# ubc-vision/DiffuseSG

Hardware: NVIDIA B200
Metric: sampled scene graphs/sec (higher is better)
Workload: dtype bf16

## Files before the change

### diffusesg_b200/csrc/gemm.cu

```cuda
#include "common.cuh"
#include "kernels.h"

namespace dsg {
namespace {

constexpr int BM = 128;
constexpr int BK = 64;
__host__ __device__ constexpr int epi_groups(int epi) { return (epi == EPI_RES_F32 || epi == EPI_F32) ? 2 : 4; }
__host__ __device__ constexpr int gemm_threads(int epi) { return 64 + 128 * epi_groups(epi); }
constexpr int A_STAGE_BYTES = BM * BK * 2;

template <int BN, bool PAIR = false>
struct Cfg {
  static constexpr int kStages = PAIR ? ((BN == 256) ? 4 : (BN == 192) ? 5 : 7) : ((BN == 256) ? 3 : (BN == 192) ? 4 : 5);
  static constexpr int B_STAGE_BYTES = (PAIR ? BN / 2 : BN) * BK * 2;
  static constexpr int STAGE_BYTES = A_STAGE_BYTES + B_STAGE_BYTES;
  static constexpr int ACC_STRIDE = (BN >= 192) ? 256 : 128;
  static constexpr uint32_t TMEM_COLS = 2 * ACC_STRIDE;
  static constexpr int STAGING_BYTES = 64 * 1024;
  static constexpr int BIAS_BYTES = 2 * BN * 4;
  static constexpr int SMEM_BYTES = 1024  + kStages * STAGE_BYTES + STAGING_BYTES + BIAS_BYTES + 256 ;
};

static_assert(Cfg<96>::SMEM_BYTES <= 227 * 1024 && Cfg<192>::SMEM_BYTES <= 227 * 1024, "shared memory budget");
// ... 159 lines not shown
      else mbar_arrive(&tempty_bar[acc]);
    };
    for (int tile = cta + acc * ncta; tile < num_tiles; tile += 2 * ncta) {
      const int mn = tile / ksplit;
      const int m_blk = PAIR ? (mn / num_n) * 2 + static_cast<int>(rank) : mn / num_n;
      const int n_blk = mn % num_n;
      const uint32_t t_row = tmem_base + (static_cast<uint32_t>(q * 32) << 16) + acc * C::ACC_STRIDE;
      if (EPI == EPI_ADJ_HEAD) {
        float* sPart = reinterpret_cast<float*>(sOut) + acc * 128 * 8;
        if (tile == cta + acc * ncta) {
          if (tig < 48) sBiasA[half * 48 + tig] = p.bias[half * 48 + tig];
          asm volatile("bar.sync %0, 128;" ::"r"(bar_id) : "memory");
        }
        const int row = m_blk * BM + r_in_tile;
        const int n_ = p.n_img, nn_ = n_ * n_;
        const int rowc = row < p.M ? row : p.M - 1;
        int b_ = rowc / nn_, ij_ = rowc - b_ * nn_;
        if (p.perm != nullptr) {
          const int ss = p.side * p.side;
          const int img = rowc / ss, rem = rowc - img * ss;
          const int ii = rem / p.side;
          b_ = p.perm[img];
          ij_ = ii * n_ + (rem - ii * p.side);
        }
        const bool real_ = b_ >= 0;
        if (!real_) b_ = 0;
        bool ok_ = false;
        float cs_ = 0.f, co_ = 1.f, xa_[8];
        if (half == 0) {
          const int i_ = ij_ / n_, j_ = ij_ - i_ * n_;
          ok_ = p.flags[b_ * n_ + i_] != 0 && p.flags[b_ * n_ + j_] != 0;
          if (p.x_adj != nullptr) {
            cs_ = p.c_skip[b_];
            co_ = p.c_out[b_];
#pragma unroll
            for (int c = 0; c < 8; ++c) xa_[c] = c < p.c_e ? p.x_adj[(static_cast<size_t>(b_) * p.c_e + c) * nn_ + ij_] : 0.f;
          }
        }
        mbar_wait(&tfull_bar[acc], acc_ph);
        tcgen05_fence_after();
        f32x2 y2[4] = {f2_splat(0.f), f2_splat(0.f), f2_splat(0.f), f2_splat(0.f)};
#pragma unroll
        for (int c0 = 0; c0 < 48; c0 += 16) {
          uint32_t r[16];
          tmem_ld_32x16(t_row + half * 48 + c0, r);
// ... 328 lines not shown
bool gemm_use_pair(long long rows, int K, int epi) {
  return epi != EPI_ADJ_HEAD && rows >= 256 && (K >= 768 || (K >= 384 && epi == EPI_BF16));
}

int launch_gemm(const CUtensorMap* tmA, const CUtensorMap* tmW, const CUtensorMap* tmO, int epi, const GemmParams& p,
                cudaStream_t st, bool pair) {
  DSG_REQUIRE(p.M > 0 && p.N > 0 && p.K > 0 && p.N % 96 == 0 && p.K % 16 == 0,
              "gemm: unsupported shape M=%d N=%d K=%d (N %% 96 == 0 and K %% 16 == 0 required)", p.M, p.N, p.K);
  DSG_REQUIRE(p.out != nullptr, "gemm: null output");
  DSG_REQUIRE(p.ksplit <= 1, "gemm: split-K (ksplit %d) is only for the MN-major weight-gradient GEMM", p.ksplit);
  const int bn = p.bn ? p.bn : gemm_block_n(p.N);
  DSG_REQUIRE(p.N % bn == 0 && (bn == 96 || bn == 192 || bn == 256), "gemm: tile width %d for N = %d", bn, p.N);
  if (epi == EPI_ADJ_HEAD) {
    DSG_REQUIRE(p.N == 96 && p.c_e >= 1 && p.c_e <= 8 && p.w2t && p.b2 && p.flags && p.n_img > 0,
                "gemm: adj-head epilogue needs N == 96, c_e <= 8 and the head tensors");
    return launch_t<96, EPI_ADJ_HEAD>(tmA, tmW, tmO, p, st);
  }
  DSG_REQUIRE(p.ldo % 8 == 0, "gemm: ldo must be a multiple of 8");
  DSG_REQUIRE(tmO != nullptr && p.ldo == p.N, "gemm: output tensor map missing or ldo != N");
  if (epi == EPI_RES_F32)
    DSG_REQUIRE(p.res == p.out, "gemm: the residual epilogue accumulates in place (res must alias out)");
  if (pair) {
    if (bn == 256) {
      switch (epi) {
        case EPI_BF16: return launch_pair<256, EPI_BF16>(tmA, tmW, tmO, p, st);
        case EPI_GELU_BF16: return launch_pair<256, EPI_GELU_BF16>(tmA, tmW, tmO, p, st);
        case EPI_RES_F32: return launch_pair<256, EPI_RES_F32>(tmA, tmW, tmO, p, st);
        case EPI_F32: return launch_pair<256, EPI_F32>(tmA, tmW, tmO, p, st);
      }
    } else if (bn == 192) {
// ... 43 lines not shown
```

### diffusesg_b200/csrc/kernels.h

```cpp
#pragma once

#include <cuda.h>
#include <cuda_bf16.h>
#include <cuda_runtime.h>
#include <stdint.h>

namespace dsg {

typedef __nv_bfloat16 bf16;

enum GemmEpi : int {
  EPI_BF16 = 0,
  EPI_GELU_BF16 = 1,
  EPI_RES_F32 = 2,
  EPI_F32 = 3,
  EPI_ADJ_HEAD = 4,
};

struct GemmParams {
  int M, N, K;
  const float* bias;
  const float* res;
  void* out;
  int ldo;
  int bn;
  int ksplit;
  int scale_rows;
  float row_scale;
  const float* w2t;
  const float* b2;
  int c_e;
  int n_img;
  const uint8_t* flags;
  const float* x_adj;
  const float* c_skip;
  const float* c_out;
  const int* perm;
  int side;
};

int make_tmap_bf16(CUtensorMap* map, const void* base, int64_t rows, int64_t cols, int box_rows);
int make_tmap_out(CUtensorMap* map, const void* base, int64_t rows, int64_t cols, int epi);

int launch_wgrad(const void* dy, const void* x, float* dw, long long tokens, int n_out, int x_cols, int out_cols, int ksplit,
                 int scale_rows, float row_scale, cudaStream_t st);

int gemm_block_n(int N);
int gemm_choose_bn(long long rows, int N, int K, int epi, bool pair);
bool gemm_use_pair(long long rows, int K, int epi);
int launch_gemm(const CUtensorMap* tmA, const CUtensorMap* tmW, const CUtensorMap* tmO, int epi, const GemmParams& p,
                cudaStream_t st, bool pair = false);

bool fused_mlp_supported(int C);
// ... 49 lines not shown
int launch_breakup_ln(const float* t, bf16* y, const float* g1, const float* b1, const float* g2, const float* b2,
                      int batch, int res, int D, cudaStream_t st, const int* tok0 = nullptr, const int* width = nullptr,
                      int sh = 0, const int* src_perm = nullptr);

int launch_cond(const float* noise_labels, long long label_stride, int n_cond, const float* w0, const float* b0, const float* w1,
                const float* b1, const float* w_film, const float* b_film, int film_total, float* emb0, float* emb1,
                float* emb, float* film, int embed, cudaStream_t st);

int launch_precond_coef(const float* sigmas, int sigma_stride, float* coef, int batch, cudaStream_t st);

int launch_node_proj(const float* node, const float* sc_node, const float* in_scale, const float* w_rc,
                     float* rc, int batch, int n, int c_n, int self_cond, int embed, cudaStream_t st);
int launch_patch_embed(const float* adj, const float* sc_adj, const float* in_scale, const uint8_t* flags,
                       const float* rc, const float* w_adj, const float* bias, const float* gamma,
                       const float* beta, const float* film, int film_ld, int film_off, int cond_uniform,
                       float* x0, int batch, int n, int c_e, int self_cond, int embed, cudaStream_t st,
                       const int* perm = nullptr, int side = 0);
int launch_node_head(const bf16* rep, const uint8_t* flags, const float* fold_t, const float* fold_b, const float* w1t,
                     const float* b1, const float* w2t, const float* b2, const float* x_node, const float* c_skip, const float* c_out,
                     float* out_node, int batch, int n, int c_n, int embed, cudaStream_t st, const int* tok0 = nullptr,
                     const int* width = nullptr, float* scratch = nullptr);


int launch_edm_pre_step(const float* adj, const float* node, const float* eps_adj, const float* eps_node,
                        const uint8_t* flags, float noise_coef, float* adj_hat, float* node_hat, int batch,
                        int c_e, int n, int c_n, cudaStream_t st);
int launch_edm_pre_step_philox(const float* adj, const float* node, const uint8_t* flags, float noise_coef,
                               unsigned long long seed, unsigned long long offset_adj, int grid_adj,
                               unsigned long long offset_node, int grid_node, const void* dev_params, float* adj_hat,
                               float* node_hat, int batch, int c_e, int n, int c_n, cudaStream_t st);
int launch_edm_post_step(const float* adj_hat, const float* node_hat, const float* d1_adj, const float* d1_node,
                         const float* d2_adj, const float* d2_node, const uint8_t* flags, float inv_t_hat,
// ... 35 lines not shown
```

### diffusesg_b200/csrc/model.cu

```cuda
#include <cstdarg>
#include <cstdio>
#include <cstdlib>
#include <cstring>
#include <map>
#include <string>
#include <tuple>
#include <vector>

#include "../../include/dsg_b200.h"
#include "common.cuh"
#include "kernels.h"

namespace dsg {

static thread_local char g_err[1024] = "";
static unsigned long long g_launches = 0;
static int g_stop_after = -1;

void set_last_error(const char* fmt, ...) {
  va_list ap;
  va_start(ap, fmt);
  vsnprintf(g_err, sizeof(g_err), fmt, ap);
  va_end(ap);
}
// ... 370 lines not shown
  std::vector<float*> skip;
  bf16 *Y, *QKV, *ATT, *H;
  size_t bytes;
};

struct Layout {
  int level = 0;
  int K = 0;
  int count[8], side[8], img0[8];
  long long tok[9];
  const int *perm = nullptr, *tok0 = nullptr, *width = nullptr;
  bool dense() const { return perm == nullptr; }
  const int* bucket_perm(int k) const { return perm != nullptr ? perm + img0[k] : nullptr; }
  long long tokens(int s) const { return tok[K] >> (2 * s); }
  long long at(int k, int s) const { return tok[k] >> (2 * s); }
};

Layout dense_layout(int B, int N) {
  Layout l;
  l.K = 1;
  l.count[0] = B; l.side[0] = N; l.img0[0] = 0;
  l.tok[0] = 0; l.tok[1] = static_cast<long long>(B) * N * N;
  return l;
}

int parse_plan(Layout& c, int level, const int32_t* tables, int table_images, int buckets, const int32_t* counts,
               const int32_t* sides, long long phantom_tok0, int G, int B, int N) {
  DSG_REQUIRE(buckets > 0 && buckets <= 8 && table_images > 0, "forward: %d buckets", buckets);
  c.level = level;
  c.K = buckets;
// ... 433 lines not shown
  bool final_ln_done = false;
  auto block = [&](const Block& b, const float* x_in, const Layout& from, const Layout& lay, bool last) -> int {
    const int* rows_map = row_map(a, from, lay);
    if (rows_map != nullptr && x_in == w.X) std::swap(w.X, w.T);
    return run_block(m, b, w, x_in, lay, rows_map, uniform, st, last, &final_ln_done);
  };
  g_prof_pass = g_prof_on && !stream_capturing(st) && (g_prof_counter++ % g_prof_stride == 0);
  struct ProfPassGuard { ~ProfPassGuard() { g_prof_pass = false; } } prof_pass_guard;
  DSG_TRY_P(PC_EMBED_HEAD, 0, 0, launch_cond(labels, label_stride, a->n_cond, m->f32("map_layer0.weight"),
                      m->f32("map_layer0.bias"), m->f32("map_layer1.weight"), m->f32("map_layer1.bias"),
                      m->at<float>(m->film_w_off), m->at<float>(m->film_b_off), m->film_total, w.emb0, w.emb1, w.emb,
                      w.film, E, st));
  DSG_TRY_P(PC_EMBED_HEAD, 0, 0, launch_node_proj(a->node, a->sc_node, c_in, m->at<float>(m->w_rc_off), w.rc, B, N, m->cfg.c_n,
                           m->cfg.self_condition, E, st));
  const Layout& l0 = stage_layout(0);
  for (int k = 0; k < l0.K; ++k) {
    const double pxk = static_cast<double>(l0.count[k]) * l0.side[k] * l0.side[k];
    DSG_TRY_P(PC_EMBED_HEAD, 0, pxk * (m->planes_adj * 4 + E * 4),
              launch_patch_embed(a->adj, a->sc_adj, c_in, a->flags, w.rc, m->at<float>(m->w_adj_off),
                                 m->f32("patch_embed.proj.bias"), m->f32("patch_embed.norm.weight"),
                                 m->f32("patch_embed.norm.bias"), w.film, m->film_total, 0, uniform, w.X + l0.tok[k] * E,
                                 l0.count[k], N, m->cfg.c_e, m->cfg.self_condition, E, st, l0.bucket_perm(k), l0.side[k]));
  }
  const Layout* xl = &l0;
  int stage_no = 0;
#define DSG_STAGE_DONE() do { if (g_stop_after >= 0 && stage_no++ == g_stop_after) return DSG_OK; } while (0)
  DSG_STAGE_DONE();
  for (int s = 0; s < m->nl; ++s) {
    const float* x_in = s == 0 ? w.X : w.skip[s - 1];
    const Layout* in = s == 0 ? xl : &stage_layout(s - 1);
    for (int j = 0; j < m->cfg.depths[s]; ++j) {
      const Layout& lay = block_layout(s, j, 0);
      DSG_TRY(block(m->blocks[m->down_first[s] + j], x_in, *in, lay, false));
      x_in = w.X;
      in = xl = &lay;
      DSG_STAGE_DONE();
    }
    if (s < m->nl - 1) {
// ... 43 lines not shown
  const long long pixels = l0.tokens(0);
  if (!l0.dense())
    DSG_CUDA_CHECK(cudaMemsetAsync(a->out_adj, 0, static_cast<size_t>(B) * m->cfg.c_e * N * N * 4, st));
  if (!final_ln_done)
    DSG_TRY_P(PC_ROW, 0, static_cast<double>(pixels) * E * 6, launch_ln(w.X, w.Y, m->f32("norm.weight"), m->f32("norm.bias"), pixels, E, st));
  GemmParams hp;
  memset(&hp, 0, sizeof(hp));
  hp.w2t = m->at<float>(m->adj_w2t_off);
  hp.b2 = m->at<float>(m->adj_b2_off);
  hp.c_e = m->cfg.c_e;
  hp.n_img = N;
  hp.flags = a->flags;
  hp.x_adj = a->mode == 1 ? a->adj : nullptr;
  hp.c_skip = c_skip;
  hp.c_out = c_out;
  for (int k = 0; k < l0.K; ++k) {
    hp.perm = l0.bucket_perm(k);
    hp.side = l0.side[k];
    DSG_TRY(gemm(m, w.Y + l0.tok[k] * E, l0.tok[k + 1] - l0.tok[k], m->adj_fc1, EPI_ADJ_HEAD, m->at<float>(m->adj_b1_off),
                 nullptr, a->out_adj, st, &hp));
  }
  DSG_TRY_P(PC_EMBED_HEAD, 0, static_cast<double>(pixels) * E * 2, launch_node_head(w.Y, a->flags, m->at<float>(m->fold_ft_off), m->at<float>(m->fold_b_off),
                           m->at<float>(m->node_w1t_off), m->f32("readout_node_mlp.fc1.bias"),
                           m->at<float>(m->node_w2t_off), m->f32("readout_node_mlp.fc2.bias"),
                           a->mode == 1 ? a->node : nullptr, c_skip, c_out, a->out_node, B, N, m->cfg.c_n, E, st,
                           l0.tok0, l0.width, 2 * E >= 128 ? w.rc : nullptr));
  return DSG_OK;
}

void dsg_launch_count_add(uint64_t n) { __atomic_fetch_add(&g_launches, static_cast<unsigned long long>(n), __ATOMIC_RELAXED); }
void dsg_debug_set_stop_after(int n_stages) { g_stop_after = n_stages; }

int dsg_profile_begin(int pass_stride) {
  DSG_REQUIRE(pass_stride >= 1, "profile_begin: stride %d", pass_stride);
  for (int c = 0; c < PC_COUNT; ++c) {
    memset(&g_prof_tot[c], 0, sizeof(g_prof_tot[c]));
// ... 245 lines not shown
```

### diffusesg_b200/csrc/rowops.cu

```cuda
#include "common.cuh"
#include "kernels.h"

namespace dsg {
namespace {

constexpr int kRowThreads = 256;
constexpr float kLnEps = 1e-5f;

DSG_DEVICE uint2 pack4_bf16(float a, float b, float c, float d) { return make_uint2(pack_bf16x2(a, b), pack_bf16x2(c, d)); }

template <int LPR>
DSG_DEVICE float group_sum(float v) {
#pragma unroll
  for (int o = LPR / 2; o > 0; o >>= 1) v += __shfl_xor_sync(0xffffffffu, v, o);
  return v;
}

template <int NV, int LPR = 32>
struct Row {
  float4 v[NV];
  DSG_DEVICE void load(const float* p, int C, int lane) {
#pragma unroll
    for (int i = 0; i < NV; ++i) {
      const int e = (lane + LPR * i) * 4;
// ... 284 lines not shown
  if (e2 >= 2 * embed) return;
  const int which = e2 / embed, e = e2 - which * embed;
  const float* w = w_rc + static_cast<size_t>(which) * cin * embed + e;
  float wr[32];
#pragma unroll
  for (int ch = 0; ch < 32; ++ch) wr[ch] = ch < cin ? w[ch * embed] : 0.f;
  for (int r = 0; r < kNodeRows && row0 + r < rows; ++r) {
    float acc = 0.f;
#pragma unroll
    for (int ch = 0; ch < 32; ++ch) acc = fmaf(wr[ch], sv[r][ch], acc);
    rc[(row0 + r) * 2 * embed + e2] = acc;
  }
}

constexpr int kPE = 96;
__global__ void __launch_bounds__(kRowThreads, 3)
patch_embed_kernel(const float* __restrict__ adj, const float* __restrict__ sc_adj, const float* __restrict__ in_scale,
                   const uint8_t* __restrict__ flags, const float* __restrict__ rc, const float* __restrict__ w_adj,
                   const float* __restrict__ bias, const float* __restrict__ gamma, const float* __restrict__ beta,
                   const float* __restrict__ film, int film_ld, int cond_uniform, float* __restrict__ x0,
                   long long pixels, int n, int c_e, int self_cond, const int* __restrict__ perm, int side) {
  constexpr int E = kPE, NT = E / 8;
  __shared__ uint4 sBf[NT][32];
  __shared__ __align__(16) float sBias[E], sGam[E], sBet[E];
  const int planes = self_cond ? 2 * c_e : c_e;
  const int lane = threadIdx.x & 31, g = lane >> 2, t = lane & 3;
  auto split2 = [](float a, float b, uint32_t& hi, uint32_t& lo) {
    const __nv_bfloat16 ah = __float2bfloat16_rn(a), bh = __float2bfloat16_rn(b);
    hi = pack_bf16x2(__bfloat162float(ah), __bfloat162float(bh));
    lo = pack_bf16x2(a - __bfloat162float(ah), b - __bfloat162float(bh));
  };
  for (int idx = threadIdx.x; idx < NT * 32; idx += kRowThreads) {
    const int nt = idx >> 5, l = idx & 31, ch = nt * 8 + (l >> 2), k0 = 2 * (l & 3);
    auto w = [&](int k) { return k < planes ? w_adj[k * E + ch] : 0.f; };
    uint4 f;
    split2(w(k0), w(k0 + 1), f.x, f.z);
    split2(w(k0 + 8), w(k0 + 9), f.y, f.w);
    sBf[nt][l] = f;
  }
  for (int i = threadIdx.x; i < E; i += kRowThreads) { sBias[i] = bias[i]; sGam[i] = gamma[i]; sBet[i] = beta[i]; }
  __syncthreads();
  const int nn = n * n;
  const long long groups = (pixels + 15) / 16;
  const long long warps_total = static_cast<long long>(gridDim.x) * (kRowThreads / 32);
  auto load_planes = [&](long long grp, float (&pv)[8], float (&scl)[2]) {
#pragma unroll
    for (int r = 0; r < 2; ++r) {
      const long long px = grp * 16 + g + 8 * r;
      const long long pc = px < pixels ? px : pixels - 1;
      int b_ = static_cast<int>(pc / nn);
      int ij_ = static_cast<int>(pc - static_cast<long long>(b_) * nn);
      if (perm != nullptr) {
        const int img = static_cast<int>(pc / (side * side));
        const int rem = static_cast<int>(pc - static_cast<long long>(img) * side * side);
        const int i_ = rem / side;
        b_ = perm[img];
        ij_ = i_ * n + (rem - i_ * side);
      }
      scl[r] = (in_scale && b_ >= 0) ? in_scale[b_] : 1.f;
      if (b_ < 0) {
#pragma unroll
        for (int h = 0; h < 4; ++h) pv[r * 4 + h] = 0.f;
        continue;
      }
#pragma unroll
      for (int h = 0; h < 4; ++h) {
        const int k = 2 * t + (h & 1) + 8 * (h >> 1);
        float a = 0.f;
        if (k < planes) {
          if (self_cond && k < c_e) {
            if (sc_adj) a = sc_adj[(static_cast<size_t>(b_) * c_e + k) * nn + ij_];
          } else {
            a = adj[(static_cast<size_t>(b_) * c_e + (self_cond ? k - c_e : k)) * nn + ij_];
          }
        }
        pv[r * 4 + h] = a;
      }
    }
  };
  const long long grp0 = static_cast<long long>(blockIdx.x) * (kRowThreads / 32) + (threadIdx.x >> 5);
  float pv_next[8], sc_next[2];
  if (grp0 < groups) load_planes(grp0, pv_next, sc_next);
  for (long long grp = grp0; grp < groups; grp += warps_total) {
    float pv[8];
#pragma unroll
    for (int k = 0; k < 8; ++k) {
      const int kk = 2 * t + (k & 1) + 8 * ((k >> 1) & 1);
      pv[k] = (self_cond && kk < c_e) ? pv_next[k] : __fmul_rn(sc_next[k >> 2], pv_next[k]);
    }
    if (grp + warps_total < groups) load_planes(grp + warps_total, pv_next, sc_next);
    long long pix[2];
    int bb[2], ij[2];
    bool valid[2], pair_ok[2];
    const float *rrow[2], *rcol[2], *fs[2];
#pragma unroll
    for (int r = 0; r < 2; ++r) {
      pix[r] = grp * 16 + g + 8 * r;
      valid[r] = pix[r] < pixels;
      const long long pc = valid[r] ? pix[r] : pixels - 1;
      bb[r] = static_cast<int>(pc / nn);
      ij[r] = static_cast<int>(pc - static_cast<long long>(bb[r]) * nn);
      if (perm != nullptr) {
        const int img = static_cast<int>(pc / (side * side));
        const int rem = static_cast<int>(pc - static_cast<long long>(img) * side * side);
        const int ii = rem / side;
        bb[r] = perm[img];
        ij[r] = ii * n + (rem - ii * side);
      }
      const int i_ = ij[r] / n, j_ = ij[r] - i_ * n;
      const int bs = bb[r] < 0 ? 0 : bb[r];
      pair_ok[r] = bb[r] >= 0 && flags[bs * n + i_] != 0 && flags[bs * n + j_] != 0;
      rrow[r] = rc + (static_cast<size_t>(bs) * n + i_) * 2 * E;
      rcol[r] = rc + (static_cast<size_t>(bs) * n + j_) * 2 * E + E;
      fs[r] = film + static_cast<size_t>(cond_uniform ? 0 : bs) * film_ld;
    }
    uint32_t a_hi[4], a_lo[4];
    split2(pv[0], pv[1], a_hi[0], a_lo[0]);
    split2(pv[4], pv[5], a_hi[1], a_lo[1]);
    split2(pv[2], pv[3], a_hi[2], a_lo[2]);
    split2(pv[6], pv[7], a_hi[3], a_lo[3]);
    float acc[NT][4];
#pragma unroll
    for (int nt = 0; nt < NT; ++nt) {
      const float2 bv = *reinterpret_cast<const float2*>(&sBias[nt * 8 + 2 * t]);
      acc[nt][0] = bv.x; acc[nt][1] = bv.y; acc[nt][2] = bv.x; acc[nt][3] = bv.y;
      const uint4 f = sBf[nt][lane];
      const uint32_t b_hi[2] = {f.x, f.y}, b_lo[2] = {f.z, f.w};
      mma_m16n8k16_bf16(acc[nt], a_lo, b_hi);
      mma_m16n8k16_bf16(acc[nt], a_hi, b_lo);
      mma_m16n8k16_bf16(acc[nt], a_hi, b_hi);
    }
    f32x2 pr[NT][2];
#pragma unroll
    for (int nt = 0; nt < NT; ++nt) {
      pr[nt][0] = f2_pack(acc[nt][0], acc[nt][1]);
      pr[nt][1] = f2_pack(acc[nt][2], acc[nt][3]);
    }
    float mean[2], rstd[2];
#pragma unroll
    for (int r = 0; r < 2; ++r) {
      if (pair_ok[r]) {
        const float2* p1 = reinterpret_cast<const float2*>(rrow[r] + 2 * t);
        const float2* p2 = reinterpret_cast<const float2*>(rcol[r] + 2 * t);
#pragma unroll
        for (int nt = 0; nt < NT; ++nt) {
          const float2 r1 = __ldg(p1 + 4 * nt), r2 = __ldg(p2 + 4 * nt);
          pr[nt][r] = f2_add(pr[nt][r], f2_add(f2_pack(r1.x, r1.y), f2_pack(r2.x, r2.y)));
        }
      }
      f32x2 s2 = pr[0][r];
#pragma unroll
      for (int nt = 1; nt < NT; ++nt) s2 = f2_add(s2, pr[nt][r]);
      float sa, sb;
      f2_unpack(s2, sa, sb);
      float sm = sa + sb;
      sm += __shfl_xor_sync(0xffffffffu, sm, 1);
      sm += __shfl_xor_sync(0xffffffffu, sm, 2);
      mean[r] = sm * (1.0f / E);
      const f32x2 nm = f2_splat(-mean[r]);
      f32x2 q2 = f2_splat(0.f);
#pragma unroll
      for (int nt = 0; nt < NT; ++nt) {
        pr[nt][r] = f2_add(pr[nt][r], nm);
        q2 = f2_fma(pr[nt][r], pr[nt][r], q2);
      }
      f2_unpack(q2, sa, sb);
      float qq = sa + sb;
      qq += __shfl_xor_sync(0xffffffffu, qq, 1);
      qq += __shfl_xor_sync(0xffffffffu, qq, 2);
      rstd[r] = rsqrtf(qq * (1.0f / E) + kLnEps);
    }
#pragma unroll
    for (int r = 0; r < 2; ++r) {
      const f32x2 rs = f2_splat(rstd[r]);
      const float2* psc = reinterpret_cast<const float2*>(fs[r] + 2 * t);
      const float2* psh = reinterpret_cast<const float2*>(fs[r] + E + 2 * t);
      float2* orow = reinterpret_cast<float2*>(x0 + pix[r] * E + 2 * t);
      if (valid[r]) {
#pragma unroll
        for (int nt = 0; nt < NT; ++nt) {
          const float2 gg = *reinterpret_cast<const float2*>(&sGam[nt * 8 + 2 * t]);
          const float2 be = *reinterpret_cast<const float2*>(&sBet[nt * 8 + 2 * t]);
          const float2 fsc = __ldg(psc + 4 * nt), fsh = __ldg(psh + 4 * nt);
          const f32x2 y = f2_fma(f2_mul(pr[nt][r], rs), f2_pack(gg.x, gg.y), f2_pack(be.x, be.y));
          const f32x2 z = f2_fma(y, f2_add(f2_pack(fsc.x, fsc.y), f2_splat(1.f)), f2_pack(fsh.x, fsh.y));
          float z0, z1, u0, u1;
          f2_unpack(z, z0, z1);
          f2_unpack(f2_mul(z, f2_splat(-1.4426950408889634f)), u0, u1);
          const f32x2 den = f2_add(f2_pack(ex2_approx(u0), ex2_approx(u1)), f2_splat(1.f));
          float d0, d1;
          f2_unpack(den, d0, d1);
          orow[4 * nt] = make_float2(z0 * rcp_approx(d0), z1 * rcp_approx(d1));
        }
      }
    }
  }
}

constexpr int kHeadRows = 8;
__global__ void __launch_bounds__(256)
node_head_kernel(const bf16* __restrict__ rep, const uint8_t* __restrict__ flags, const float* __restrict__ fold_t,
                 const float* __restrict__ fold_b, const float* __restrict__ w1t,
                 const float* __restrict__ b1, const float* __restrict__ w2t, const float* __restrict__ b2,
                 const float* __restrict__ x_node, const float* __restrict__ c_skip, const float* __restrict__ c_out,
                 float* __restrict__ out_node, long long rows, int n, int c_n, int embed, const int* __restrict__ tok0,
                 const int* __restrict__ width) {
  __shared__ float va[kHeadRows][128];
  __shared__ float vb[kHeadRows][128];
  __shared__ float frac[kHeadRows];
  const int warp = threadIdx.x >> 5, lane = threadIdx.x & 31;
  const long long row0 = static_cast<long long>(blockIdx.x) * kHeadRows;
// ... 311 lines not shown
  return DSG_OK;
}

int launch_node_proj(const float* node, const float* sc_node, const float* in_scale, const float* w_rc, float* rc,
                     int batch, int n, int c_n, int self_cond, int embed, cudaStream_t st) {
  DSG_REQUIRE(2 * embed <= 1024 && (self_cond ? 2 : 1) * c_n <= 32, "node_proj: embed %d, c_n %d", embed, c_n);
  const long long rows = static_cast<long long>(batch) * n;
  node_proj_kernel<<<static_cast<unsigned>((rows + kNodeRows - 1) / kNodeRows), 2 * embed, 0, st>>>(
      node, sc_node, in_scale, w_rc, rc, batch, n, c_n, self_cond, embed);
  DSG_LAUNCH_CHECK();
  return DSG_OK;
}

int launch_patch_embed(const float* adj, const float* sc_adj, const float* in_scale, const uint8_t* flags,
                       const float* rc, const float* w_adj, const float* bias, const float* gamma, const float* beta,
                       const float* film, int film_ld, int film_off, int cond_uniform, float* x0, int batch, int n,
                       int c_e, int self_cond, int embed, cudaStream_t st, const int* perm, int side) {
  DSG_REQUIRE(embed == 96, "patch_embed: embed_dim %d (only 96 is built)", embed);
  const long long pixels = perm != nullptr ? static_cast<long long>(batch) * side * side : static_cast<long long>(batch) * n * n;
  DSG_REQUIRE((self_cond ? 2 : 1) * c_e <= 16, "patch_embed: %d adjacency planes (max 16)", (self_cond ? 2 : 1) * c_e);
  long long blocks = (pixels / 16 + 7) / 8;
  if (blocks > 148 * 3) blocks = 148 * 3;
  patch_embed_kernel<<<static_cast<unsigned>(blocks), kRowThreads, 0, st>>>(adj, sc_adj, in_scale, flags, rc, w_adj,
                                                                           bias, gamma, beta, film + film_off, film_ld,
                                                                           cond_uniform, x0, pixels, n, c_e, self_cond,
                                                                           perm, side);
  DSG_LAUNCH_CHECK();
  return DSG_OK;
}

int launch_node_head(const bf16* rep, const uint8_t* flags, const float* fold_t, const float* fold_b, const float* w1t,
                     const float* b1, const float* w2t, const float* b2, const float* x_node, const float* c_skip,
                     const float* c_out, float* out_node, int batch, int n, int c_n, int embed, cudaStream_t st,
                     const int* tok0, const int* width, float* scratch) {
  DSG_REQUIRE(embed <= 128 && embed % 4 == 0 && c_n <= 128, "node_head: embed %d c_n %d", embed, c_n);
  const long long rows = static_cast<long long>(batch) * n;
  if (embed == 96 && c_n <= 32 && n <= 64 && scratch != nullptr) {
    node_pool_kernel<<<static_cast<unsigned>((rows + 7) / 8), 256, 0, st>>>(rep, flags, scratch, rows, n, tok0, width);
    DSG_LAUNCH_CHECK();
    constexpr int smem = (96 * 32 + (2 * 96 + 1) * kMlpRows) * 4;
    static PerDeviceOnce configured;
// ... 15 lines not shown
```

Measured before the change: 66.63.

## Rewrite patch embed on tcgen05 with TMA store and single bucketed launch

Replaces the mma.sync patch-embed kernel with a persistent tcgen05/TMEM kernel. It keeps a split-bf16 weight in shared memory, gathers column node projections with cp.async, and writes output tiles through TMA bulk stores. A BucketTable lets both patch embed and the adjacency-head GEMM cover all size buckets in one launch instead of one launch per bucket. This cuts launch count and moves the tiny-K projection to the newer tensor core path. In exchange it adds far more shared memory, one CTA per SM, and more complex synchronisation for a small-K GEMM.

```diff
diff --git a/diffusesg_b200/csrc/gemm.cu b/diffusesg_b200/csrc/gemm.cu
--- a/diffusesg_b200/csrc/gemm.cu
+++ b/diffusesg_b200/csrc/gemm.cu
@@ -197,21 +197,14 @@
         }
         const int row = m_blk * BM + r_in_tile;
         const int n_ = p.n_img, nn_ = n_ * n_;
-        const int rowc = row < p.M ? row : p.M - 1;
-        int b_ = rowc / nn_, ij_ = rowc - b_ * nn_;
-        if (p.perm != nullptr) {
-          const int ss = p.side * p.side;
-          const int img = rowc / ss, rem = rowc - img * ss;
-          const int ii = rem / p.side;
-          b_ = p.perm[img];
-          ij_ = ii * n_ + (rem - ii * p.side);
-        }
+        int i_, j_;
+        int b_ = bucket_pixel(p.rows, row < p.M ? row : p.M - 1, i_, j_);
+        const int ij_ = i_ * n_ + j_;
         const bool real_ = b_ >= 0;
         if (!real_) b_ = 0;
         bool ok_ = false;
         float cs_ = 0.f, co_ = 1.f, xa_[8];
         if (half == 0) {
-          const int i_ = ij_ / n_, j_ = ij_ - i_ * n_;
           ok_ = p.flags[b_ * n_ + i_] != 0 && p.flags[b_ * n_ + j_] != 0;
           if (p.x_adj != nullptr) {
             cs_ = p.c_skip[b_];
@@ -570,6 +563,8 @@
   if (epi == EPI_ADJ_HEAD) {
     DSG_REQUIRE(p.N == 96 && p.c_e >= 1 && p.c_e <= 8 && p.w2t && p.b2 && p.flags && p.n_img > 0,
                 "gemm: adj-head epilogue needs N == 96, c_e <= 8 and the head tensors");
+    DSG_REQUIRE(p.rows.K >= 1 && p.rows.K <= 8 && p.rows.tok[p.rows.K] == p.M,
+                "gemm: adj-head bucket table of %d buckets does not cover the %d rows", p.rows.K, p.M);
     return launch_t<96, EPI_ADJ_HEAD>(tmA, tmW, tmO, p, st);
   }
   DSG_REQUIRE(p.ldo % 8 == 0, "gemm: ldo must be a multiple of 8");
diff --git a/diffusesg_b200/csrc/kernels.h b/diffusesg_b200/csrc/kernels.h
--- a/diffusesg_b200/csrc/kernels.h
+++ b/diffusesg_b200/csrc/kernels.h
@@ -8,6 +8,26 @@
 namespace dsg {
 
 typedef __nv_bfloat16 bf16;
+
+struct BucketTable {
+  int K;
+  int side[8], img0[8];
+  long long tok[9];
+  const int* perm;
+};
+
+__host__ __device__ __forceinline__ int bucket_pixel(const BucketTable& t, long long row, int& i, int& j) {
+  long long t0 = t.tok[0];
+  int side = t.side[0], img0 = t.img0[0];
+#pragma unroll
+  for (int k = 1; k < 8; ++k)
+    if (k < t.K && row >= t.tok[k]) { t0 = t.tok[k]; side = t.side[k]; img0 = t.img0[k]; }
+  const int local = static_cast<int>(row - t0), ss = side * side;
+  const int img = local / ss, rem = local - img * ss;
+  i = rem / side;
+  j = rem - i * side;
+  return t.perm != nullptr ? t.perm[img0 + img] : img;
+}
 
 enum GemmEpi : int {
   EPI_BF16 = 0,
@@ -35,8 +55,7 @@
   const float* x_adj;
   const float* c_skip;
   const float* c_out;
-  const int* perm;
-  int side;
+  BucketTable rows;
 };
 
 int make_tmap_bf16(CUtensorMap* map, const void* base, int64_t rows, int64_t cols, int box_rows);
@@ -116,8 +135,7 @@
 int launch_patch_embed(const float* adj, const float* sc_adj, const float* in_scale, const uint8_t* flags,
                        const float* rc, const float* w_adj, const float* bias, const float* gamma,
                        const float* beta, const float* film, int film_ld, int film_off, int cond_uniform,
-                       float* x0, int batch, int n, int c_e, int self_cond, int embed, cudaStream_t st,
-                       const int* perm = nullptr, int side = 0);
+                       float* x0, const BucketTable& rows, int n, int c_e, int self_cond, int embed, cudaStream_t st);
 int launch_node_head(const bf16* rep, const uint8_t* flags, const float* fold_t, const float* fold_b, const float* w1t,
                      const float* b1, const float* w2t, const float* b2, const float* x_node, const float* c_skip, const float* c_out,
                      float* out_node, int batch, int n, int c_n, int embed, cudaStream_t st, const int* tok0 = nullptr,
diff --git a/diffusesg_b200/csrc/model.cu b/diffusesg_b200/csrc/model.cu
--- a/diffusesg_b200/csrc/model.cu
+++ b/diffusesg_b200/csrc/model.cu
@@ -408,6 +408,15 @@
   const int* bucket_perm(int k) const { return perm != nullptr ? perm + img0[k] : nullptr; }
   long long tokens(int s) const { return tok[K] >> (2 * s); }
   long long at(int k, int s) const { return tok[k] >> (2 * s); }
+  BucketTable rows() const {
+    BucketTable t;
+    memset(&t, 0, sizeof(t));
+    t.K = K;
+    for (int k = 0; k < K; ++k) { t.side[k] = side[k]; t.img0[k] = img0[k]; t.tok[k] = tok[k]; }
+    t.tok[K] = tok[K];
+    t.perm = perm;
+    return t;
+  }
 };
 
 Layout dense_layout(int B, int N) {
@@ -871,14 +880,12 @@
   DSG_TRY_P(PC_EMBED_HEAD, 0, 0, launch_node_proj(a->node, a->sc_node, c_in, m->at<float>(m->w_rc_off), w.rc, B, N, m->cfg.c_n,
                            m->cfg.self_condition, E, st));
   const Layout& l0 = stage_layout(0);
-  for (int k = 0; k < l0.K; ++k) {
-    const double pxk = static_cast<double>(l0.count[k]) * l0.side[k] * l0.side[k];
-    DSG_TRY_P(PC_EMBED_HEAD, 0, pxk * (m->planes_adj * 4 + E * 4),
-              launch_patch_embed(a->adj, a->sc_adj, c_in, a->flags, w.rc, m->at<float>(m->w_adj_off),
-                                 m->f32("patch_embed.proj.bias"), m->f32("patch_embed.norm.weight"),
-                                 m->f32("patch_embed.norm.bias"), w.film, m->film_total, 0, uniform, w.X + l0.tok[k] * E,
-                                 l0.count[k], N, m->cfg.c_e, m->cfg.self_condition, E, st, l0.bucket_perm(k), l0.side[k]));
-  }
+  const double px0 = static_cast<double>(l0.tokens(0));
+  DSG_TRY_P(PC_EMBED_HEAD, 0, px0 * (m->planes_adj * 4 + E * 4),
+            launch_patch_embed(a->adj, a->sc_adj, c_in, a->flags, w.rc, m->at<float>(m->w_adj_off),
+                               m->f32("patch_embed.proj.bias"), m->f32("patch_embed.norm.weight"),
+                               m->f32("patch_embed.norm.bias"), w.film, m->film_total, 0, uniform, w.X, l0.rows(), N,
+                               m->cfg.c_e, m->cfg.self_condition, E, st));
   const Layout* xl = &l0;
   int stage_no = 0;
 #define DSG_STAGE_DONE() do { if (g_stop_after >= 0 && stage_no++ == g_stop_after) return DSG_OK; } while (0)
@@ -952,12 +959,8 @@
   hp.x_adj = a->mode == 1 ? a->adj : nullptr;
   hp.c_skip = c_skip;
   hp.c_out = c_out;
-  for (int k = 0; k < l0.K; ++k) {
-    hp.perm = l0.bucket_perm(k);
-    hp.side = l0.side[k];
-    DSG_TRY(gemm(m, w.Y + l0.tok[k] * E, l0.tok[k + 1] - l0.tok[k], m->adj_fc1, EPI_ADJ_HEAD, m->at<float>(m->adj_b1_off),
-                 nullptr, a->out_adj, st, &hp));
-  }
+  hp.rows = l0.rows();
+  DSG_TRY(gemm(m, w.Y, pixels, m->adj_fc1, EPI_ADJ_HEAD, m->at<float>(m->adj_b1_off), nullptr, a->out_adj, st, &hp));
   DSG_TRY_P(PC_EMBED_HEAD, 0, static_cast<double>(pixels) * E * 2, launch_node_head(w.Y, a->flags, m->at<float>(m->fold_ft_off), m->at<float>(m->fold_b_off),
                            m->at<float>(m->node_w1t_off), m->f32("readout_node_mlp.fc1.bias"),
                            m->at<float>(m->node_w2t_off), m->f32("readout_node_mlp.fc2.bias"),
diff --git a/diffusesg_b200/csrc/rowops.cu b/diffusesg_b200/csrc/rowops.cu
--- a/diffusesg_b200/csrc/rowops.cu
+++ b/diffusesg_b200/csrc/rowops.cu
@@ -1,3 +1,5 @@
+#include <algorithm>
+
 #include "common.cuh"
 #include "kernels.h"
 
@@ -322,187 +324,252 @@
 }
 
 constexpr int kPE = 96;
-__global__ void __launch_bounds__(kRowThreads, 3)
-patch_embed_kernel(const float* __restrict__ adj, const float* __restrict__ sc_adj, const float* __restrict__ in_scale,
-                   const uint8_t* __restrict__ flags, const float* __restrict__ rc, const float* __restrict__ w_adj,
-                   const float* __restrict__ bias, const float* __restrict__ gamma, const float* __restrict__ beta,
-                   const float* __restrict__ film, int film_ld, int cond_uniform, float* __restrict__ x0,
-                   long long pixels, int n, int c_e, int self_cond, const int* __restrict__ perm, int side) {
-  constexpr int E = kPE, NT = E / 8;
-  __shared__ uint4 sBf[NT][32];
-  __shared__ __align__(16) float sBias[E], sGam[E], sBet[E];
+constexpr int kEmbedGroups = 2;
+constexpr int kEmbedThreads = 128 * kEmbedGroups;
+constexpr int kEmbedTile = 128 * 128;
+constexpr int kEmbedStage = 3 * 128 * 32 * 4;
+constexpr int kEmbedSmem = 1024  + kPE * 128  + kEmbedGroups * (kEmbedTile + kEmbedStage) +
+                           3 * kPE * 4  + 64 ;
+static_assert(kEmbedSmem <= 227 * 1024, "shared memory budget");
+
+struct EmbedPixel {
+  float pv[16];
+  float scl;
+  int b, i, j;
+  bool ok;
+};
+
+__global__ void __launch_bounds__(kEmbedThreads, 1)
+patch_embed_tc_kernel(const __grid_constant__ CUtensorMap tmX, const float* __restrict__ adj,
+                      const float* __restrict__ sc_adj, const float* __restrict__ in_scale,
+                      const uint8_t* __restrict__ flags, const float* __restrict__ rc, const float* __restrict__ w_adj,
+                      const float* __restrict__ bias, const float* __restrict__ gamma, const float* __restrict__ beta,
+                      const float* __restrict__ film, int film_ld, int cond_uniform, const BucketTable rows_tab,
+                      int n, int c_e, int self_cond) {
+  constexpr int E = kPE;
+  extern __shared__ uint8_t smem_raw[];
+  uint8_t* smem = smem_raw + ((1024u - (smem_u32(smem_raw) & 1023u)) & 1023u);
+  uint8_t* sW = smem;
+  uint8_t* sA0 = sW + E * 128;
+  uint8_t* sOut0 = sA0 + kEmbedGroups * kEmbedTile;
+  float* sBias = reinterpret_cast<float*>(sOut0 + kEmbedGroups * kEmbedStage);
+  float* sGam = sBias + E;
+  float* sBet = sGam + E;
+  uint64_t* mma_bar = reinterpret_cast<uint64_t*>(sBet + E);
+  uint32_t* tmem_slot = reinterpret_cast<uint32_t*>(mma_bar + kEmbedGroups);
+
+  const int warp = uniform_warp_id();
+  const int lane = threadIdx.x & 31;
+  const int grp = warp >> 2, q = warp & 3;
+  const int r = q * 32 + lane;
   const int planes = self_cond ? 2 * c_e : c_e;
-  const int lane = threadIdx.x & 31, g = lane >> 2, t = lane & 3;
-  auto split2 = [](float a, float b, uint32_t& hi, uint32_t& lo) {
-    const __nv_bfloat16 ah = __float2bfloat16_rn(a), bh = __float2bfloat16_rn(b);
-    hi = pack_bf16x2(__bfloat162float(ah), __bfloat162float(bh));
-    lo = pack_bf16x2(a - __bfloat162float(ah), b - __bfloat162float(bh));
+  auto put_row = [](uint8_t* row_base, int row, const float (&v)[16]) {
+    uint32_t h[8], l[8];
+#pragma unroll
+    for (int k = 0; k < 8; ++k) {
+      h[k] = pack_bf16x2(v[2 * k], v[2 * k + 1]);
+      l[k] = pack_bf16x2(v[2 * k] - __uint_as_float(h[k] << 16), v[2 * k + 1] - __uint_as_float(h[k] & 0xffff0000u));
+    }
+    const int sw = row & 7;
+    *reinterpret_cast<uint4*>(row_base + ((0 ^ sw) << 4)) = make_uint4(h[0], h[1], h[2], h[3]);
+    *reinterpret_cast<uint4*>(row_base + ((1 ^ sw) << 4)) = make_uint4(h[4], h[5], h[6], h[7]);
+    *reinterpret_cast<uint4*>(row_base + ((2 ^ sw) << 4)) = make_uint4(l[0], l[1], l[2], l[3]);
+    *reinterpret_cast<uint4*>(row_base + ((3 ^ sw) << 4)) = make_uint4(l[4], l[5], l[6], l[7]);
   };
-  for (int idx = threadIdx.x; idx < NT * 32; idx += kRowThreads) {
-    const int nt = idx >> 5, l = idx & 31, ch = nt * 8 + (l >> 2), k0 = 2 * (l & 3);
-    auto w = [&](int k) { return k < planes ? w_adj[k * E + ch] : 0.f; };
-    uint4 f;
-    split2(w(k0), w(k0 + 1), f.x, f.z);
-    split2(w(k0 + 8), w(k0 + 9), f.y, f.w);
-    sBf[nt][l] = f;
-  }
-  for (int i = threadIdx.x; i < E; i += kRowThreads) { sBias[i] = bias[i]; sGam[i] = gamma[i]; sBet[i] = beta[i]; }
-  __syncthreads();
-  const int nn = n * n;
-  const long long groups = (pixels + 15) / 16;
-  const long long warps_total = static_cast<long long>(gridDim.x) * (kRowThreads / 32);
-  auto load_planes = [&](long long grp, float (&pv)[8], float (&scl)[2]) {
-#pragma unroll
-    for (int r = 0; r < 2; ++r) {
-      const long long px = grp * 16 + g + 8 * r;
-      const long long pc = px < pixels ? px : pixels - 1;
-      int b_ = static_cast<int>(pc / nn);
-      int ij_ = static_cast<int>(pc - static_cast<long long>(b_) * nn);
-      if (perm != nullptr) {
-        const int img = static_cast<int>(pc / (side * side));
-        const int rem = static_cast<int>(pc - static_cast<long long>(img) * side * side);
-        const int i_ = rem / side;
-        b_ = perm[img];
-        ij_ = i_ * n + (rem - i_ * side);
-      }
-      scl[r] = (in_scale && b_ >= 0) ? in_scale[b_] : 1.f;
-      if (b_ < 0) {
-#pragma unroll
-        for (int h = 0; h < 4; ++h) pv[r * 4 + h] = 0.f;
-        continue;
-      }
-#pragma unroll
-      for (int h = 0; h < 4; ++h) {
-        const int k = 2 * t + (h & 1) + 8 * (h >> 1);
-        float a = 0.f;
-        if (k < planes) {
-          if (self_cond && k < c_e) {
-            if (sc_adj) a = sc_adj[(static_cast<size_t>(b_) * c_e + k) * nn + ij_];
-          } else {
-            a = adj[(static_cast<size_t>(b_) * c_e + (self_cond ? k - c_e : k)) * nn + ij_];
-          }
-        }
-        pv[r * 4 + h] = a;
-      }
-    }
-  };
-  const long long grp0 = static_cast<long long>(blockIdx.x) * (kRowThreads / 32) + (threadIdx.x >> 5);
-  float pv_next[8], sc_next[2];
-  if (grp0 < groups) load_planes(grp0, pv_next, sc_next);
-  for (long long grp = grp0; grp < groups; grp += warps_total) {
-    float pv[8];
-#pragma unroll
-    for (int k = 0; k < 8; ++k) {
-      const int kk = 2 * t + (k & 1) + 8 * ((k >> 1) & 1);
-      pv[k] = (self_cond && kk < c_e) ? pv_next[k] : __fmul_rn(sc_next[k >> 2], pv_next[k]);
-    }
-    if (grp + warps_total < groups) load_planes(grp + warps_total, pv_next, sc_next);
-    long long pix[2];
-    int bb[2], ij[2];
-    bool valid[2], pair_ok[2];
-    const float *rrow[2], *rcol[2], *fs[2];
-#pragma unroll
-    for (int r = 0; r < 2; ++r) {
-      pix[r] = grp * 16 + g + 8 * r;
-      valid[r] = pix[r] < pixels;
-      const long long pc = valid[r] ? pix[r] : pixels - 1;
-      bb[r] = static_cast<int>(pc / nn);
-      ij[r] = static_cast<int>(pc - static_cast<long long>(bb[r]) * nn);
-      if (perm != nullptr) {
-        const int img = static_cast<int>(pc / (side * side));
-        const int rem = static_cast<int>(pc - static_cast<long long>(img) * side * side);
-        const int ii = rem / side;
-        bb[r] = perm[img];
-        ij[r] = ii * n + (rem - ii * side);
-      }
-      const int i_ = ij[r] / n, j_ = ij[r] - i_ * n;
-      const int bs = bb[r] < 0 ? 0 : bb[r];
-      pair_ok[r] = bb[r] >= 0 && flags[bs * n + i_] != 0 && flags[bs * n + j_] != 0;
-      rrow[r] = rc + (static_cast<size_t>(bs) * n + i_) * 2 * E;
-      rcol[r] = rc + (static_cast<size_t>(bs) * n + j_) * 2 * E + E;
-      fs[r] = film + static_cast<size_t>(cond_uniform ? 0 : bs) * film_ld;
-    }
-    uint32_t a_hi[4], a_lo[4];
-    split2(pv[0], pv[1], a_hi[0], a_lo[0]);
-    split2(pv[4], pv[5], a_hi[1], a_lo[1]);
-    split2(pv[2], pv[3], a_hi[2], a_lo[2]);
-    split2(pv[6], pv[7], a_hi[3], a_lo[3]);
-    float acc[NT][4];
-#pragma unroll
-    for (int nt = 0; nt < NT; ++nt) {
-      const float2 bv = *reinterpret_cast<const float2*>(&sBias[nt * 8 + 2 * t]);
-      acc[nt][0] = bv.x; acc[nt][1] = bv.y; acc[nt][2] = bv.x; acc[nt][3] = bv.y;
-      const uint4 f = sBf[nt][lane];
-      const uint32_t b_hi[2] = {f.x, f.y}, b_lo[2] = {f.z, f.w};
-      mma_m16n8k16_bf16(acc[nt], a_lo, b_hi);
-      mma_m16n8k16_bf16(acc[nt], a_hi, b_lo);
-      mma_m16n8k16_bf16(acc[nt], a_hi, b_hi);
-    }
-    f32x2 pr[NT][2];
-#pragma unroll
-    for (int nt = 0; nt < NT; ++nt) {
-      pr[nt][0] = f2_pack(acc[nt][0], acc[nt][1]);
-      pr[nt][1] = f2_pack(acc[nt][2], acc[nt][3]);
-    }
-    float mean[2], rstd[2];
-#pragma unroll
-    for (int r = 0; r < 2; ++r) {
-      if (pair_ok[r]) {
-        const float2* p1 = reinterpret_cast<const float2*>(rrow[r] + 2 * t);
-        const float2* p2 = reinterpret_cast<const float2*>(rcol[r] + 2 * t);
-#pragma unroll
-        for (int nt = 0; nt < NT; ++nt) {
-          const float2 r1 = __ldg(p1 + 4 * nt), r2 = __ldg(p2 + 4 * nt);
-          pr[nt][r] = f2_add(pr[nt][r], f2_add(f2_pack(r1.x, r1.y), f2_pack(r2.x, r2.y)));
+
+  if (threadIdx.x < E) {
+    float v[16];
+#pragma unroll
+    for (int k = 0; k < 16; ++k) v[k] = k < planes ? w_adj[k * E + threadIdx.x] : 0.f;
+    put_row(sW + threadIdx.x * 128, threadIdx.x, v);
+  }
+  for (int i = threadIdx.x; i < E; i += kEmbedThreads) { sBias[i] = bias[i]; sGam[i] = gamma[i]; sBet[i] = beta[i]; }
+  if (warp == 0) {
+    if (lane < kEmbedGroups) mbar_init(&mma_bar[lane], 1);
+    fence_barrier_init();
+    tmem_alloc<kEmbedGroups * 128>(tmem_slot);
+  }
+  if (threadIdx.x == 0) tma_prefetch_desc(&tmX);
+  fence_proxy_async_smem();
+  tcgen05_fence_before();
+  __syncthreads();
+  tcgen05_fence_after();
+  const uint32_t tmem_base = uniform_u32(*tmem_slot);
+  const uint32_t t_row = tmem_base + (static_cast<uint32_t>(q * 32) << 16) + grp * 128;
+
+  const long long rows = rows_tab.tok[rows_tab.K];
+  const long long tiles = (rows + 127) / 128;
+  const long long step = static_cast<long long>(kEmbedGroups) * gridDim.x;
+  auto load = [&](long long tile, EmbedPixel& px) {
+    const long long row = tile * 128 + r;
+    px.i = px.j = 0;
+    px.b = row < rows ? bucket_pixel(rows_tab, row, px.i, px.j) : -1;
+    const int bs = px.b < 0 ? 0 : px.b;
+    px.ok = px.b >= 0 && flags[bs * n + px.i] != 0 && flags[bs * n + px.j] != 0;
+    px.scl = (in_scale && px.b >= 0) ? in_scale[px.b] : 1.f;
+    const int nn = n * n, ij = px.i * n + px.j;
+    const float* sc_b = sc_adj != nullptr ? sc_adj + static_cast<size_t>(bs) * c_e * nn + ij : nullptr;
+    const float* adj_b = adj + static_cast<size_t>(bs) * c_e * nn + ij - (self_cond ? c_e * nn : 0);
+#pragma unroll
+    for (int k = 0; k < 16; ++k) {
+      float a = 0.f;
+      if (px.b >= 0 && k < planes) {
+        if (self_cond && k < c_e) {
+          if (sc_b != nullptr) a = sc_b[k * nn];
+        } else {
+          a = adj_b[k * nn];
         }
       }
-      f32x2 s2 = pr[0][r];
-#pragma unroll
-      for (int nt = 1; nt < NT; ++nt) s2 = f2_add(s2, pr[nt][r]);
-      float sa, sb;
-      f2_unpack(s2, sa, sb);
-      float sm = sa + sb;
-      sm += __shfl_xor_sync(0xffffffffu, sm, 1);
-      sm += __shfl_xor_sync(0xffffffffu, sm, 2);
-      mean[r] = sm * (1.0f / E);
-      const f32x2 nm = f2_splat(-mean[r]);
-      f32x2 q2 = f2_splat(0.f);
-#pragma unroll
-      for (int nt = 0; nt < NT; ++nt) {
-        pr[nt][r] = f2_add(pr[nt][r], nm);
-        q2 = f2_fma(pr[nt][r], pr[nt][r], q2);
+      px.pv[k] = a;
+    }
+  };
+
+  uint8_t* sA = sA0 + grp * kEmbedTile;
+  uint8_t* sOut = sOut0 + grp * kEmbedStage;
+  const int bar_id = 1 + grp;
+  const bool issuer = r == 0;
+  uint32_t ph = 0;
+  EmbedPixel px;
+  long long tile = blockIdx.x + static_cast<long long>(grp) * gridDim.x;
+  if (tile < tiles) load(tile, px);
+  for (; tile < tiles; tile += step) {
+    {
+      float v[16];
+#pragma unroll
+      for (int k = 0; k < 16; ++k) v[k] = (self_cond && k < c_e) ? px.pv[k] : __fmul_rn(px.scl, px.pv[k]);
+      put_row(sA + r * 128, r, v);
+    }
+    fence_proxy_async_smem();
+    tcgen05_fence_before();
+    if (issuer) asm volatile("cp.async.bulk.wait_group.read 0;" ::: "memory");
+    asm volatile("bar.sync %0, 128;" ::"r"(bar_id) : "memory");
+    if (q == 0) {
+      tcgen05_fence_after();
+      if (elect_one()) {
+        constexpr uint32_t idesc = umma_idesc_bf16(E);
+        const uint64_t da = umma_desc_sw128(smem_u32(sA)), db = umma_desc_sw128(smem_u32(sW));
+        const uint32_t d = tmem_base + grp * 128;
+        umma_bf16_ss(d, da + 2, db, idesc, 0u);
+        umma_bf16_ss(d, da, db + 2, idesc, 1u);
+        umma_bf16_ss(d, da, db, idesc, 1u);
+        umma_commit(&mma_bar[grp]);
       }
-      f2_unpack(q2, sa, sb);
-      float qq = sa + sb;
-      qq += __shfl_xor_sync(0xffffffffu, qq, 1);
-      qq += __shfl_xor_sync(0xffffffffu, qq, 2);
-      rstd[r] = rsqrtf(qq * (1.0f / E) + kLnEps);
-    }
-#pragma unroll
-    for (int r = 0; r < 2; ++r) {
-      const f32x2 rs = f2_splat(rstd[r]);
-      const float2* psc = reinterpret_cast<const float2*>(fs[r] + 2 * t);
-      const float2* psh = reinterpret_cast<const float2*>(fs[r] + E + 2 * t);
-      float2* orow = reinterpret_cast<float2*>(x0 + pix[r] * E + 2 * t);
-      if (valid[r]) {
-#pragma unroll
-        for (int nt = 0; nt < NT; ++nt) {
-          const float2 gg = *reinterpret_cast<const float2*>(&sGam[nt * 8 + 2 * t]);
-          const float2 be = *reinterpret_cast<const float2*>(&sBet[nt * 8 + 2 * t]);
-          const float2 fsc = __ldg(psc + 4 * nt), fsh = __ldg(psh + 4 * nt);
-          const f32x2 y = f2_fma(f2_mul(pr[nt][r], rs), f2_pack(gg.x, gg.y), f2_pack(be.x, be.y));
-          const f32x2 z = f2_fma(y, f2_add(f2_pack(fsc.x, fsc.y), f2_splat(1.f)), f2_pack(fsh.x, fsh.y));
+      __syncwarp();
+    }
+    const bool pair_ok = px.ok;
+    const int bs = px.b < 0 ? 0 : px.b;
+    const int film_row = (cond_uniform ? 0 : bs) * film_ld;
+    const float4* rrow = reinterpret_cast<const float4*>(rc + (static_cast<size_t>(bs) * n + px.i) * 2 * E);
+    {
+      const uint32_t okm = __ballot_sync(0xffffffffu, pair_ok);
+      const int nj = bs * n + px.j;
+#pragma unroll 8
+      for (int t = 0; t < 32; ++t) {
+        const int rj = __shfl_sync(0xffffffffu, nj, t);
+        const int row = q * 32 + t;
+        if (((okm >> t) & 1u) && lane < E / 4)
+          asm volatile("cp.async.cg.shared.global [%0], [%1], 16;"
+                       ::"r"(smem_u32(sOut + (lane >> 3) * (128 * 128) + row * 128 + (((lane & 7) ^ (row & 7)) << 4))),
+                       "l"(reinterpret_cast<const float4*>(rc + static_cast<size_t>(rj) * 2 * E + E) + lane)
+                       : "memory");
+      }
+      asm volatile("cp.async.commit_group;" ::: "memory");
+    }
+    const long long cur = tile;
+
+    mbar_wait(&mma_bar[grp], ph);
+    ph ^= 1;
+    tcgen05_fence_after();
+    uint32_t acc[3][32];
+    tmem_ld_32x32(t_row, acc[0]);
+    tmem_ld_32x32(t_row + 32, acc[1]);
+    tmem_ld_32x32(t_row + 64, acc[2]);
+    tmem_ld_wait();
+    f32x2 x[E / 2];
+#pragma unroll
+    for (int c = 0; c < E / 4; ++c) {
+      const float4 bb = *reinterpret_cast<const float4*>(&sBias[4 * c]);
+      const uint32_t* a4 = &acc[c / 8][(4 * c) % 32];
+      x[2 * c] = f2_add(f2_pack(__uint_as_float(a4[0]), __uint_as_float(a4[1])), f2_pack(bb.x, bb.y));
+      x[2 * c + 1] = f2_add(f2_pack(__uint_as_float(a4[2]), __uint_as_float(a4[3])), f2_pack(bb.z, bb.w));
+    }
+    asm volatile("cp.async.wait_group 0;" ::: "memory");
+    __syncwarp();
+    if (pair_ok) {
+#pragma unroll
+      for (int c = 0; c < E / 4; ++c) {
+        if (c % 8 == 0) asm volatile("" ::: "memory");
+        const float4 r1 = __ldg(rrow + c);
+        const float4 r2 = *reinterpret_cast<const float4*>(sOut + (c >> 3) * (128 * 128) + r * 128 + (((c & 7) ^ (r & 7)) << 4));
+        x[2 * c] = f2_add(x[2 * c], f2_add(f2_pack(r1.x, r1.y), f2_pack(r2.x, r2.y)));
+        x[2 * c + 1] = f2_add(x[2 * c + 1], f2_add(f2_pack(r1.z, r1.w), f2_pack(r2.z, r2.w)));
+      }
+    }
+    if (tile + step < tiles) load(tile + step, px);
+    f32x2 s2 = x[0];
+#pragma unroll
+    for (int c = 1; c < E / 2; ++c) s2 = f2_add(s2, x[c]);
+    float sa, sb;
+    f2_unpack(s2, sa, sb);
+    const f32x2 nm = f2_splat(-(sa + sb) * (1.0f / E));
+    f32x2 q2 = f2_splat(0.f);
+#pragma unroll
+    for (int c = 0; c < E / 2; ++c) {
+      x[c] = f2_add(x[c], nm);
+      q2 = f2_fma(x[c], x[c], q2);
+    }
+    f2_unpack(q2, sa, sb);
+    const f32x2 rs = f2_splat(rsqrtf((sa + sb) * (1.0f / E) + kLnEps));
+#pragma unroll
+    for (int ch = 0; ch < 3; ++ch) {
+      uint8_t* rowp = sOut + ch * (128 * 128) + r * 128;
+#pragma unroll
+      for (int u = 0; u < 8; ++u) {
+        if (u % 4 == 0) asm volatile("" ::: "memory");
+        const int c4 = ch * 8 + u;
+        const float4 gg = *reinterpret_cast<const float4*>(&sGam[4 * c4]);
+        const float4 be = *reinterpret_cast<const float4*>(&sBet[4 * c4]);
+        const float4 sc = __ldg(reinterpret_cast<const float4*>(film + film_row) + c4);
+        const float4 sh = __ldg(reinterpret_cast<const float4*>(film + film_row + E) + c4);
+        float o[4];
+#pragma unroll
+        for (int h = 0; h < 2; ++h) {
+          const f32x2 g2 = h ? f2_pack(gg.z, gg.w) : f2_pack(gg.x, gg.y);
+          const f32x2 b2 = h ? f2_pack(be.z, be.w) : f2_pack(be.x, be.y);
+          const f32x2 s2c = h ? f2_pack(sc.z, sc.w) : f2_pack(sc.x, sc.y);
+          const f32x2 h2 = h ? f2_pack(sh.z, sh.w) : f2_pack(sh.x, sh.y);
+          const f32x2 y = f2_fma(f2_mul(x[2 * c4 + h], rs), g2, b2);
+          const f32x2 z = f2_fma(y, f2_add(s2c, f2_splat(1.f)), h2);
           float z0, z1, u0, u1;
           f2_unpack(z, z0, z1);
           f2_unpack(f2_mul(z, f2_splat(-1.4426950408889634f)), u0, u1);
           const f32x2 den = f2_add(f2_pack(ex2_approx(u0), ex2_approx(u1)), f2_splat(1.f));
           float d0, d1;
           f2_unpack(den, d0, d1);
-          orow[4 * nt] = make_float2(z0 * rcp_approx(d0), z1 * rcp_approx(d1));
+          o[2 * h] = z0 * rcp_approx(d0);
+          o[2 * h + 1] = z1 * rcp_approx(d1);
         }
+        *reinterpret_cast<float4*>(rowp + ((u ^ (r & 7)) << 4)) = make_float4(o[0], o[1], o[2], o[3]);
       }
     }
-  }
+    fence_proxy_async_smem();
+    asm volatile("bar.sync %0, 128;" ::"r"(bar_id) : "memory");
+    if (issuer) {
+      const int row0 = static_cast<int>(cur * 128);
+#pragma unroll
+      for (int ch = 0; ch < 3; ++ch)
+        asm volatile("cp.async.bulk.tensor.2d.global.shared::cta.bulk_group [%0, {%2, %3}], [%1];"
+                     ::"l"(reinterpret_cast<uint64_t>(&tmX)), "r"(smem_u32(sOut + ch * (128 * 128))), "r"(ch * 32),
+                     "r"(row0)
+                     : "memory");
+      asm volatile("cp.async.bulk.commit_group;" ::: "memory");
+    }
+  }
+  if (issuer) asm volatile("cp.async.bulk.wait_group 0;" ::: "memory");
+  tcgen05_fence_before();
+  __syncthreads();
+  tcgen05_fence_after();
+  if (warp == 0) tmem_dealloc<kEmbedGroups * 128>(tmem_base);
 }
 
 constexpr int kHeadRows = 8;
@@ -844,17 +911,25 @@
 
 int launch_patch_embed(const float* adj, const float* sc_adj, const float* in_scale, const uint8_t* flags,
                        const float* rc, const float* w_adj, const float* bias, const float* gamma, const float* beta,
-                       const float* film, int film_ld, int film_off, int cond_uniform, float* x0, int batch, int n,
-                       int c_e, int self_cond, int embed, cudaStream_t st, const int* perm, int side) {
-  DSG_REQUIRE(embed == 96, "patch_embed: embed_dim %d (only 96 is built)", embed);
-  const long long pixels = perm != nullptr ? static_cast<long long>(batch) * side * side : static_cast<long long>(batch) * n * n;
+                       const float* film, int film_ld, int film_off, int cond_uniform, float* x0,
+                       const BucketTable& rows, int n, int c_e, int self_cond, int embed, cudaStream_t st) {
+  DSG_REQUIRE(embed == kPE, "patch_embed: embed_dim %d (only 96 is built)", embed);
   DSG_REQUIRE((self_cond ? 2 : 1) * c_e <= 16, "patch_embed: %d adjacency planes (max 16)", (self_cond ? 2 : 1) * c_e);
-  long long blocks = (pixels / 16 + 7) / 8;
-  if (blocks > 148 * 3) blocks = 148 * 3;
-  patch_embed_kernel<<<static_cast<unsigned>(blocks), kRowThreads, 0, st>>>(adj, sc_adj, in_scale, flags, rc, w_adj,
-                                                                           bias, gamma, beta, film + film_off, film_ld,
-                                                                           cond_uniform, x0, pixels, n, c_e, self_cond,
-                                                                           perm, side);
+  DSG_REQUIRE(rows.K >= 1 && rows.K <= 8 && rows.tok[rows.K] > 0 && rows.tok[rows.K] < (1ll << 31),
+              "patch_embed: %d buckets", rows.K);
+  DSG_REQUIRE(film_ld % 4 == 0 && film_off % 4 == 0 && (reinterpret_cast<uintptr_t>(film) & 15) == 0 &&
+                  (reinterpret_cast<uintptr_t>(rc) & 15) == 0,
+              "patch_embed: FiLM / node planes not 16-byte aligned (ld %d, offset %d)", film_ld, film_off);
+  CUtensorMap tmX;
+  if (int e = make_tmap_out(&tmX, x0, rows.tok[rows.K], kPE, EPI_F32)) return e;
+  static PerDeviceOnce configured;
+  if (configured.first())
+    DSG_CUDA_CHECK(cudaFuncSetAttribute(patch_embed_tc_kernel, cudaFuncAttributeMaxDynamicSharedMemorySize, kEmbedSmem));
+  const long long tiles = (rows.tok[rows.K] + 127) / 128;
+  const long long ctas = std::min<long long>((tiles + kEmbedGroups - 1) / kEmbedGroups, device_sm_count());
+  patch_embed_tc_kernel<<<static_cast<unsigned>(ctas), kEmbedThreads, kEmbedSmem, st>>>(
+      tmX, adj, sc_adj, in_scale, flags, rc, w_adj, bias, gamma, beta, film + film_off, film_ld, cond_uniform, rows, n,
+      c_e, self_cond);
   DSG_LAUNCH_CHECK();
   return DSG_OK;
 }
```

New measurement: 66.69 (median of 6 runs). No clear change (+0.1%).
